# tencent-ailab/V-Express

Measured on NVIDIA H100. Metric: frames_per_sec_512x512_25step, higher is better.
Workload: dtype bf16

## Files before the change

### v-express_b200/csrc/vx_flash_attn.cu

```cuda
#include "vx_host.h"
#include "vx_ptx.cuh"

namespace vx {

constexpr int kFaRows = 64;
constexpr int kFaThreads = 128;

struct FaArgs {
  int Nq, Nk, hd, kv_div, stages;
  float scale_log2;
  __nv_bfloat16* out;
  long long ldo;
};

template <int HDP>
__global__ void __launch_bounds__(kFaThreads)
flash_attn_wgmma_kernel(const __grid_constant__ CUtensorMap mapQ, const __grid_constant__ CUtensorMap mapK,
                        const __grid_constant__ CUtensorMap mapV, const FaArgs p) {
  constexpr int kTile = kFaRows * HDP * 2;
  extern __shared__ uint8_t smem_raw[];
  uint8_t* smem = reinterpret_cast<uint8_t*>((reinterpret_cast<uintptr_t>(smem_raw) + 127) & ~uintptr_t(127));
  uint8_t* sQ = smem;
  uint8_t* sK = sQ + kTile;
  uint8_t* sV = sK + p.stages * kTile;
  uint64_t* q_full = reinterpret_cast<uint64_t*>(sV + p.stages * kTile);
  uint64_t* kv_full = q_full + 1;

  const int warp = threadIdx.x >> 5, lane = threadIdx.x & 31;
  const int q_tile = blockIdx.x, head = blockIdx.y, bq = blockIdx.z;
  const int T = (p.Nk + kFaRows - 1) / kFaRows;
  if (HDP > p.hd) {
    uint4* z = reinterpret_cast<uint4*>(sQ);
    for (int i = threadIdx.x; i < (1 + 2 * p.stages) * kTile / 16; i += blockDim.x) z[i] = make_uint4(0, 0, 0, 0);
  }
  if (threadIdx.x == 0) {
    mbar_init(q_full, 1);
    for (int s = 0; s < p.stages; ++s) mbar_init(&kv_full[s], 1);
    fence_barrier_init();
  }
  fence_proxy_async_smem();
  __syncthreads();
  pdl_wait();

  const int col_chunk = head * p.hd / 8;
  const int kv_row0 = (bq / p.kv_div) * p.Nk;
  auto load_kv = [&](int j) {
    const int st = j % p.stages;
    mbar_expect_tx(&kv_full[st], 2 * kFaRows * p.hd * 2);
    tma_load_3d(sK + st * kTile, &mapK, &kv_full[st], 0, kv_row0 + j * kFaRows, col_chunk);
    tma_load_3d(sV + st * kTile, &mapV, &kv_full[st], 0, kv_row0 + j * kFaRows, col_chunk);
  };
  if (threadIdx.x == 0) {
    tma_prefetch_desc(&mapQ);
    tma_prefetch_desc(&mapK);
    tma_prefetch_desc(&mapV);
    mbar_expect_tx(q_full, kFaRows * p.hd * 2);
    tma_load_3d(sQ, &mapQ, q_full, 0, bq * p.Nq + q_tile * kFaRows, col_chunk);
    for (int j = 0; j < p.stages && j < T; ++j) load_kv(j);
  }

  const uint64_t dq = make_smem_desc(smem_u32(sQ), kFaRows * 16, 128, SWZ_NONE);
  const float c = p.scale_log2;
  float o[HDP / 2];
#pragma unroll
  for (int i = 0; i < HDP / 2; ++i) o[i] = 0.f;
  float m_run[2] = {-INFINITY, -INFINITY}, l[2] = {0.f, 0.f};
  const int cq = (lane & 3) * 2;
  mbar_wait(q_full, 0);
  for (int j = 0; j < T; ++j) {
    const int st = j % p.stages;
    mbar_wait(&kv_full[st], (uint32_t)((j / p.stages) & 1));
    float s[32];
    const uint64_t dk = make_smem_desc(smem_u32(sK + st * kTile), kFaRows * 16, 128, SWZ_NONE);
    wgmma_fence();
#pragma unroll
    for (int k = 0; k < HDP / 16; ++k) Wgmma<64>::ss<0, 0>(s, dq + (uint64_t)(k * 128), dk + (uint64_t)(k * 128), k);
    wgmma_commit();
    wgmma_wait<0>();
    wgmma_fence_regs(s);
    if ((j + 1) * kFaRows > p.Nk) {
#pragma unroll
      for (int i = 0; i < 32; ++i)
        if (j * kFaRows + (i >> 2) * 8 + cq + (i & 1) >= p.Nk) s[i] = -INFINITY;
    }
    float alpha[2], mc[2];
#pragma unroll
    for (int h = 0; h < 2; ++h) {
      float mx = -INFINITY;
#pragma unroll
      for (int g = 0; g < 8; ++g) mx = fmaxf(mx, fmaxf(s[4 * g + 2 * h], s[4 * g + 2 * h + 1]));
      mx = fmaxf(mx, __shfl_xor_sync(0xffffffffu, mx, 1));
      mx = fmaxf(mx, __shfl_xor_sync(0xffffffffu, mx, 2));
      const float m_new = fmaxf(m_run[h], mx);
      alpha[h] = m_run[h] == -INFINITY ? 0.f : exp2f((m_run[h] - m_new) * c);
      m_run[h] = m_new;
      mc[h] = m_new * c;
      l[h] *= alpha[h];
    }
#pragma unroll
    for (int i = 0; i < HDP / 2; ++i) o[i] *= alpha[(i >> 1) & 1];
    uint32_t pa[4][4];
#pragma unroll
    for (int i = 0; i < 32; i += 2) {
      const int h = (i >> 1) & 1;
      const float e0 = exp2f(fmaf(s[i], c, -mc[h])), e1 = exp2f(fmaf(s[i + 1], c, -mc[h]));
      l[h] += e0 + e1;
      pa[i >> 3][(i >> 1) & 3] = pack_bf16(e0, e1);
    }
    const uint64_t dv = make_smem_desc(smem_u32(sV + st * kTile), 128, kFaRows * 16, SWZ_NONE);
    wgmma_fence();
#pragma unroll
    for (int k = 0; k < kFaRows / 16; ++k) Wgmma<HDP>::template rs<1>(o, pa[k], dv + (uint64_t)(k * 16), 1);
    wgmma_commit();
    wgmma_wait<0>();
    wgmma_fence_regs(o);
    __syncthreads();
    if (threadIdx.x == 0 && j + p.stages < T) load_kv(j + p.stages);
  }
#pragma unroll
  for (int h = 0; h < 2; ++h) {
    float lt = l[h];
    lt += __shfl_xor_sync(0xffffffffu, lt, 1);
    lt += __shfl_xor_sync(0xffffffffu, lt, 2);
    const float inv = 1.f / lt;
    const int qrow = q_tile * kFaRows + warp * 16 + (lane >> 2) + 8 * h;
    if (qrow < p.Nq) {
      __nv_bfloat16* op = p.out + ((long long)bq * p.Nq + qrow) * p.ldo + head * p.hd;
#pragma unroll
      for (int g = 0; g < HDP / 8; ++g)
        if (g * 8 + cq < p.hd)
          *reinterpret_cast<uint32_t*>(op + g * 8 + cq) = pack_bf16(o[4 * g + 2 * h] * inv, o[4 * g + 2 * h + 1] * inv);
    }
  }
}

constexpr int kFaPipeMaxHd = 56;
constexpr int kFaPipeStages = 4;

template <int HD, int NCONS>
__global__ void __launch_bounds__(128 * (NCONS + 1), 2)
flash_attn_pipe_kernel(const __grid_constant__ CUtensorMap mapQ, const __grid_constant__ CUtensorMap mapK,
                       const __grid_constant__ CUtensorMap mapV, const FaArgs p) {
  constexpr int HDP = (HD + 15) / 16 * 16;
  constexpr int kTile = kFaRows * HDP * 2;
  extern __shared__ uint8_t smem_raw[];
  uint8_t* smem = reinterpret_cast<uint8_t*>((reinterpret_cast<uintptr_t>(smem_raw) + 127) & ~uintptr_t(127));
  uint8_t* sQ = smem;
  uint8_t* sK = sQ + NCONS * kTile;
  uint8_t* sV = sK + p.stages * kTile;
  uint64_t* q_full = reinterpret_cast<uint64_t*>(sV + p.stages * kTile);
  uint64_t* kv_full = q_full + 1;
  uint64_t* kv_empty = kv_full + p.stages;

  const int warp = threadIdx.x >> 5, lane = threadIdx.x & 31;
  const int q_tile = blockIdx.x, head = blockIdx.y, bq = blockIdx.z;
  const int T = (p.Nk + kFaRows - 1) / kFaRows;
  if (HDP > HD) {
    uint4* z = reinterpret_cast<uint4*>(sQ);
    for (int i = threadIdx.x; i < (NCONS + 2 * p.stages) * kTile / 16; i += blockDim.x) z[i] = make_uint4(0, 0, 0, 0);
  }
  if (threadIdx.x == 0) {
    mbar_init(q_full, 1);
    for (int s = 0; s < p.stages; ++s) {
      mbar_init(&kv_full[s], 1);
      mbar_init(&kv_empty[s], 4 * NCONS);
    }
    fence_barrier_init();
  }
  fence_proxy_async_smem();
  __syncthreads();
  pdl_wait();

  const int col_chunk = head * HD / 8;
  if (warp < 4) {
    if (NCONS == 2) setmaxnreg_dec<24>();
    if (warp == 0 && lane == 0) {
      tma_prefetch_desc(&mapQ);
      tma_prefetch_desc(&mapK);
      tma_prefetch_desc(&mapV);
      mbar_expect_tx(q_full, NCONS * kFaRows * HD * 2);
      for (int w = 0; w < NCONS; ++w)
        tma_load_3d(sQ + w * kTile, &mapQ, q_full, 0, bq * p.Nq + (q_tile * NCONS + w) * kFaRows, col_chunk);
      const int kv_row0 = (bq / p.kv_div) * p.Nk;
      int st = 0;
      uint32_t phase = 0;
      for (int j = 0; j < T; ++j) {
        if (j >= p.stages) mbar_wait(&kv_empty[st], phase ^ 1);
        mbar_expect_tx(&kv_full[st], 2 * kFaRows * HD * 2);
        tma_load_3d(sK + st * kTile, &mapK, &kv_full[st], 0, kv_row0 + j * kFaRows, col_chunk);
        tma_load_3d(sV + st * kTile, &mapV, &kv_full[st], 0, kv_row0 + j * kFaRows, col_chunk);
        if (++st == p.stages) {
          st = 0;
          phase ^= 1;
        }
      }
    }
    return;
  }
  if (NCONS == 2) setmaxnreg_inc<104>();
  const int wg = (warp >> 2) - 1;
  const uint64_t dq = make_smem_desc(smem_u32(sQ + wg * kTile), kFaRows * 16, 128, SWZ_NONE);
  const float c = p.scale_log2;
  const int cq = (lane & 3) * 2;
  float o[HD / 2], s[32];
  uint32_t pa[4][4];
#pragma unroll
  for (int i = 0; i < HD / 2; ++i) o[i] = 0.f;
  float m_run[2] = {-INFINITY, -INFINITY}, l[2] = {0.f, 0.f}, alpha[2];

  auto issue_s = [&](int st) {
    const uint64_t dk = make_smem_desc(smem_u32(sK + st * kTile), kFaRows * 16, 128, SWZ_NONE);
#pragma unroll
    for (int k = 0; k < HDP / 16; ++k) Wgmma<64>::ss<0, 0>(s, dq + (uint64_t)(k * 128), dk + (uint64_t)(k * 128), k);
    wgmma_commit();
  };
  auto softmax = [&](int j) {
    if ((j + 1) * kFaRows > p.Nk) {
#pragma unroll
      for (int i = 0; i < 32; ++i)
        if (j * kFaRows + (i >> 2) * 8 + cq + (i & 1) >= p.Nk) s[i] = -INFINITY;
    }
    float mc[2];
#pragma unroll
    for (int h = 0; h < 2; ++h) {
      float mx = -INFINITY;
#pragma unroll
      for (int g = 0; g < 8; ++g) mx = fmaxf(mx, fmaxf(s[4 * g + 2 * h], s[4 * g + 2 * h + 1]));
      mx = fmaxf(mx, __shfl_xor_sync(0xffffffffu, mx, 1));
      mx = fmaxf(mx, __shfl_xor_sync(0xffffffffu, mx, 2));
      const float m_new = fmaxf(m_run[h], mx);
      alpha[h] = ex2_ftz(__fmul_rn(__fsub_rn(m_run[h], m_new), c));
      m_run[h] = m_new;
      mc[h] = __fmul_rn(m_new, c);
    }
#pragma unroll
    for (int i = 0; i < 32; i += 2) {
      const int h = (i >> 1) & 1;
      s[i] = ex2_ftz(__fmaf_rn(s[i], c, -mc[h]));
      s[i + 1] = ex2_ftz(__fmaf_rn(s[i + 1], c, -mc[h]));
      const float e = __fadd_rn(s[i], s[i + 1]);
      l[h] = i < 4 ? __fmaf_rn(l[h], alpha[h], e) : __fadd_rn(l[h], e);
    }
  };
  auto pack = [&]() {
#pragma unroll
    for (int i = 0; i < 32; i += 2) pa[i >> 3][(i >> 1) & 3] = pack_bf16(s[i], s[i + 1]);
  };

  mbar_wait(q_full, 0);
  mbar_wait(&kv_full[0], 0);
  wgmma_fence();
  issue_s(0);
  wgmma_wait<0>();
  wgmma_fence_regs(s);
  softmax(0);
  pack();
  auto issue_pv = [&](int st) {
    const uint64_t dv = make_smem_desc(smem_u32(sV + st * kTile), 128, kFaRows * 16, SWZ_NONE);
#pragma unroll
    for (int k = 0; k < kFaRows / 16; ++k) Wgmma<HD>::template rs<1>(o, pa[k], dv + (uint64_t)(k * 16), 1);
    wgmma_commit();
  };
  auto pv_done = [&](int st) {
    wgmma_fence_regs(o);
#pragma unroll
    for (int k = 0; k < 4; ++k) wgmma_fence_regs(pa[k]);
    if (lane == 0) mbar_arrive(&kv_empty[st]);
  };
  int st = 0;
  uint32_t phase = 0;
  for (int j = 0; j + 1 < T; ++j) {
    int st1 = st + 1;
    uint32_t phase1 = phase;
    if (st1 == p.stages) {
      st1 = 0;
      phase1 ^= 1;
    }
    mbar_wait(&kv_full[st1], phase1);
    wgmma_fence();
    issue_s(st1);
    issue_pv(st);
    wgmma_wait<1>();
    wgmma_fence_regs(s);
    softmax(j + 1);
    wgmma_wait<0>();
    pv_done(st);
#pragma unroll
    for (int i = 0; i < HD / 2; ++i) o[i] = __fmul_rn(o[i], alpha[(i >> 1) & 1]);
    pack();
    st = st1;
    phase = phase1;
  }
  wgmma_fence();
  issue_pv(st);
  wgmma_wait<0>();
  pv_done(st);
#pragma unroll
  for (int h = 0; h < 2; ++h) {
    float lt = l[h];
    lt += __shfl_xor_sync(0xffffffffu, lt, 1);
    lt += __shfl_xor_sync(0xffffffffu, lt, 2);
    const float inv = 1.f / lt;
    const int qrow = (q_tile * NCONS + wg) * kFaRows + (warp & 3) * 16 + (lane >> 2) + 8 * h;
    if (qrow < p.Nq) {
      __nv_bfloat16* op = p.out + ((long long)bq * p.Nq + qrow) * p.ldo + head * HD;
#pragma unroll
      for (int g = 0; g < HD / 8; ++g)
        *reinterpret_cast<uint32_t*>(op + g * 8 + cq) = pack_bf16(o[4 * g + 2 * h] * inv, o[4 * g + 2 * h + 1] * inv);
    }
  }
}

template <auto Kernel>
static cudaError_t launch_fa(dim3 grid, int threads, size_t smem, cudaStream_t st, const CUtensorMap& mQ,
                             const CUtensorMap& mK, const CUtensorMap& mV, const FaArgs& a) {
  static bool configured = false;
  if (!configured) {
    const cudaError_t e = cudaFuncSetAttribute(Kernel, cudaFuncAttributeMaxDynamicSharedMemorySize, 227 * 1024);
    if (e != cudaSuccess) return e;
    configured = true;
  }
  return launch_k(Kernel, grid, dim3(threads), smem, st, mQ, mK, mV, a);
}

struct GaArgs {
  const __nv_bfloat16* q; long long ldq;
  const __nv_bfloat16* k; long long ldk;
  const __nv_bfloat16* v; long long ldv;
  __nv_bfloat16* out; long long ldo;
  int Bq, Nq, Nk, heads, hd, kv_div;
  float scale;
};

__global__ void __launch_bounds__(128) generic_attn_kernel(const GaArgs p) {
  pdl_enter();
  extern __shared__ float sc_all[];
  const int warp = threadIdx.x >> 5, lane = threadIdx.x & 31;
  float* sc = sc_all + warp * p.Nk;
  const long long item = (long long)blockIdx.x * 4 + warp;
  const long long total = (long long)p.Bq * p.heads * p.Nq;
  if (item >= total) return;
  const int qi = (int)(item % p.Nq);
  const int head = (int)((item / p.Nq) % p.heads);
  const int b = (int)(item / ((long long)p.Nq * p.heads));
  const __nv_bfloat16* qp = p.q + ((long long)b * p.Nq + qi) * p.ldq + head * p.hd;
  const long long kv0 = (long long)(b / p.kv_div) * p.Nk;
  float mx = -INFINITY;
  for (int j = lane; j < p.Nk; j += 32) {
    const __nv_bfloat16* kp = p.k + (kv0 + j) * p.ldk + head * p.hd;
    float acc = 0.f;
    for (int c = 0; c < p.hd; c += 2) {
      const float2 a = __bfloat1622float2(*reinterpret_cast<const __nv_bfloat162*>(qp + c));
      const float2 bb = __bfloat1622float2(*reinterpret_cast<const __nv_bfloat162*>(kp + c));
      acc += a.x * bb.x + a.y * bb.y;
    }
    acc *= p.scale;
    sc[j] = acc;
    mx = fmaxf(mx, acc);
  }
  for (int o = 16; o; o >>= 1) mx = fmaxf(mx, __shfl_xor_sync(0xffffffffu, mx, o));
  float sum = 0.f;
  for (int j = lane; j < p.Nk; j += 32) {
    const float e = __expf(sc[j] - mx);
    sc[j] = e;
    sum += e;
  }
  for (int o = 16; o; o >>= 1) sum += __shfl_xor_sync(0xffffffffu, sum, o);
  __syncwarp();
  const float inv = 1.f / sum;
  for (int c = lane * 2; c < p.hd; c += 64) {
    float o0 = 0.f, o1 = 0.f;
    for (int j = 0; j < p.Nk; ++j) {
      const float2 vv = __bfloat1622float2(*reinterpret_cast<const __nv_bfloat162*>(p.v + (kv0 + j) * p.ldv + head * p.hd + c));
      o0 += sc[j] * vv.x;
      o1 += sc[j] * vv.y;
    }
    *reinterpret_cast<__nv_bfloat162*>(p.out + ((long long)b * p.Nq + qi) * p.ldo + head * p.hd + c) =
        __floats2bfloat162_rn(o0 * inv, o1 * inv);
  }
}

}

using namespace vx;

static bool& fa_v1() {
  static bool v = getenv("VX_FA_V1") != nullptr;
  return v;
}
extern "C" void vx_flash_reload_env() { fa_v1() = getenv("VX_FA_V1") != nullptr; }

extern "C" int vx_flash_attention(const void* q, long long ldq, const void* k, long long ldk, const void* v,
                                  long long ldv, void* out, long long ldo, int Bq, int Nq, int Bkv, int Nk, int heads,
                                  int hd, int kv_div, void* stream) {
  VX_REQUIRE(hd % 8 == 0 && hd <= 256, "vx_flash_attention: hd=%d unsupported", hd);
  VX_REQUIRE(ldq % 8 == 0 && ldk % 8 == 0 && ldv % 8 == 0 && ldo % 8 == 0, "vx_flash_attention: ld must be %%8");
  VX_REQUIRE(kv_div >= 1 && (Bq + kv_div - 1) / kv_div <= Bkv, "vx_flash_attention: kv_div=%d Bq=%d Bkv=%d", kv_div, Bq, Bkv);
  if (Nk < 16 || Nk % 16 != 0) {
    VX_REQUIRE(Nk * 4 * 4 <= 48 * 1024, "vx_flash_attention: Nk=%d not a multiple of 16 and too long for the fallback", Nk);
    GaArgs g{(const __nv_bfloat16*)q, ldq, (const __nv_bfloat16*)k, ldk, (const __nv_bfloat16*)v, ldv,
             (__nv_bfloat16*)out, ldo, Bq, Nq, Nk, heads, hd, kv_div, 1.0f / sqrtf((float)hd)};
    const long long items = (long long)Bq * heads * Nq;
    launch_k(generic_attn_kernel, dim3((unsigned)((items + 3) / 4)), dim3(128), (size_t)Nk * 4 * 4, (cudaStream_t)stream, g);
    VX_CHECK_CUDA(cudaGetLastError());
    return 0;
  }
  const int hdp = (hd + 15) / 16 * 16;
  const bool pipe = hd <= kFaPipeMaxHd && !fa_v1();
  const int ncons = pipe && Nq > kFaRows ? 2 : 1;
  const int stages = pipe ? kFaPipeStages : hdp > 96 ? 2 : 3;
  const size_t smem = (size_t)(ncons + 2 * stages) * kFaRows * hdp * 2 + 128 + 128;
  CUtensorMap mQ, mK, mV;
  const void* ptrs[3] = {q, k, v};
  const long long lds[3] = {ldq, ldk, ldv};
  const long long rows[3] = {(long long)Bq * Nq, (long long)Bkv * Nk, (long long)Bkv * Nk};
  CUtensorMap* maps[3] = {&mQ, &mK, &mV};
  for (int i = 0; i < 3; ++i) {
    uint64_t dims[3] = {8, (uint64_t)rows[i], (uint64_t)lds[i] / 8};
    uint64_t str[2] = {(uint64_t)lds[i] * 2, 16};
    uint32_t box[3] = {8, (uint32_t)kFaRows, (uint32_t)hd / 8};
    if (make_tmap_bf16(maps[i], ptrs[i], 3, dims, str, box, CU_TENSOR_MAP_SWIZZLE_NONE)) return 1;
  }
  FaArgs a{};
  a.Nq = Nq; a.Nk = Nk; a.hd = hd; a.kv_div = kv_div; a.stages = stages;
  a.scale_log2 = 1.4426950408889634f / sqrtf((float)hd);
  a.out = (__nv_bfloat16*)out; a.ldo = ldo;
  const dim3 grid((Nq + ncons * kFaRows - 1) / (ncons * kFaRows), heads, Bq);
  if (pipe) {
    const cudaStream_t cs = (cudaStream_t)stream;
    cudaError_t e;
    switch (hd) {
#define VX_FA_CASE(H)                                                                                       \
    case H:                                                                                                 \
      if (ncons == 2) e = launch_fa<flash_attn_pipe_kernel<H, 2>>(grid, 384, smem, cs, mQ, mK, mV, a);         \
      else e = launch_fa<flash_attn_pipe_kernel<H, 1>>(grid, 256, smem, cs, mQ, mK, mV, a);                    \
      break;
      VX_FA_CASE(8) VX_FA_CASE(16) VX_FA_CASE(24) VX_FA_CASE(32) VX_FA_CASE(40) VX_FA_CASE(48) VX_FA_CASE(56)
#undef VX_FA_CASE
      default: return fail("vx_flash_attention: hd=%d unsupported", hd);
    }
    VX_CHECK_CUDA(e);
    VX_CHECK_CUDA(cudaGetLastError());
    return 0;
  }
  switch (hdp) {
#define VX_FA_CASE(H) \
    case H: VX_CHECK_CUDA(launch_fa<flash_attn_wgmma_kernel<H>>(grid, kFaThreads, smem, (cudaStream_t)stream, mQ, mK, mV, a)); break;
    VX_FA_CASE(16) VX_FA_CASE(32) VX_FA_CASE(48) VX_FA_CASE(64) VX_FA_CASE(80) VX_FA_CASE(96) VX_FA_CASE(112) VX_FA_CASE(128)
    VX_FA_CASE(144) VX_FA_CASE(160) VX_FA_CASE(176) VX_FA_CASE(192) VX_FA_CASE(208) VX_FA_CASE(224) VX_FA_CASE(240)
    VX_FA_CASE(256)
#undef VX_FA_CASE
    default: return fail("vx_flash_attention: hd=%d unsupported", hd);
  }
  VX_CHECK_CUDA(cudaGetLastError());
  return 0;
}
```

Before: 5.443.

## Extend warp-specialized flash attention to hd 80/160 and add three-consumer ping-pong path

Extends the producer/consumer TMA-pipelined attention kernel to head dims 80 and 160, which are typical of UNet attention layers in this model. For small head dims with long queries it uses three consumer warpgroups, double-buffering the score registers so the next QK^T GEMM is already issued while softmax runs on the current tile. Register budgets, CTAs per SM and ring depth are now computed from the head dim and consumer count instead of being fixed. The cost is higher register pressure and shared-memory use, and occupancy drops to one CTA per SM for the multi-consumer variants.

```diff
diff --git a/v-express_b200/csrc/vx_flash_attn.cu b/v-express_b200/csrc/vx_flash_attn.cu
--- a/v-express_b200/csrc/vx_flash_attn.cu
+++ b/v-express_b200/csrc/vx_flash_attn.cu
@@ -134,11 +134,24 @@
   }
 }
 
-constexpr int kFaPipeMaxHd = 56;
-constexpr int kFaPipeStages = 4;
+constexpr bool fa_pipe_hd(int hd) { return hd % 8 == 0 && (hd <= 56 || hd == 80 || hd == 160); }
+constexpr int fa_pipe_ncons(int hd, int Nq) { return Nq <= kFaRows ? 1 : hd <= 56 ? 3 : 2; }
+constexpr int fa_pipe_ctas(int ncons) { return ncons == 1 ? 2 : 1; }
+constexpr int fa_pipe_consumer_regs(int ncons) {
+  const int pool = 65536 / (fa_pipe_ctas(ncons) * 128 * (ncons + 1)) / 8 * 8 * (ncons + 1);
+  const int r = (pool - 24) / ncons / 8 * 8;
+  return r < 232 ? r : 232;
+}
+constexpr int fa_pipe_stages(int hd, int ncons) {
+  const int tile = kFaRows * ((hd + 15) / 16 * 16) * 2;
+  const int per_cta = 228 * 1024 / fa_pipe_ctas(ncons) - 1024 - 256;
+  const int s = (per_cta - ncons * tile) / (2 * tile);
+  return s < 4 ? s : 4;
+}
+static_assert(fa_pipe_stages(160, 1) >= 2 && fa_pipe_stages(160, 2) == 4 && fa_pipe_stages(56, 3) == 4, "ring depth");
 
 template <int HD, int NCONS>
-__global__ void __launch_bounds__(128 * (NCONS + 1), 2)
+__global__ void __launch_bounds__(128 * (NCONS + 1), fa_pipe_ctas(NCONS))
 flash_attn_pipe_kernel(const __grid_constant__ CUtensorMap mapQ, const __grid_constant__ CUtensorMap mapK,
                        const __grid_constant__ CUtensorMap mapV, const FaArgs p) {
   constexpr int HDP = (HD + 15) / 16 * 16;
@@ -173,7 +186,7 @@
 
   const int col_chunk = head * HD / 8;
   if (warp < 4) {
-    if (NCONS == 2) setmaxnreg_dec<24>();
+    setmaxnreg_dec<24>();
     if (warp == 0 && lane == 0) {
       tma_prefetch_desc(&mapQ);
       tma_prefetch_desc(&mapK);
@@ -197,7 +210,7 @@
     }
     return;
   }
-  if (NCONS == 2) setmaxnreg_inc<104>();
+  setmaxnreg_inc<fa_pipe_consumer_regs(NCONS)>();
   const int wg = (warp >> 2) - 1;
   const uint64_t dq = make_smem_desc(smem_u32(sQ + wg * kTile), kFaRows * 16, 128, SWZ_NONE);
   const float c = p.scale_log2;
@@ -208,13 +221,13 @@
   for (int i = 0; i < HD / 2; ++i) o[i] = 0.f;
   float m_run[2] = {-INFINITY, -INFINITY}, l[2] = {0.f, 0.f}, alpha[2];
 
-  auto issue_s = [&](int st) {
+  auto issue_s = [&](float (&s)[32], int st) {
     const uint64_t dk = make_smem_desc(smem_u32(sK + st * kTile), kFaRows * 16, 128, SWZ_NONE);
 #pragma unroll
     for (int k = 0; k < HDP / 16; ++k) Wgmma<64>::ss<0, 0>(s, dq + (uint64_t)(k * 128), dk + (uint64_t)(k * 128), k);
     wgmma_commit();
   };
-  auto softmax = [&](int j) {
+  auto softmax = [&](float (&s)[32], int j) {
     if ((j + 1) * kFaRows > p.Nk) {
 #pragma unroll
       for (int i = 0; i < 32; ++i)
@@ -242,33 +255,101 @@
       l[h] = i < 4 ? __fmaf_rn(l[h], alpha[h], e) : __fadd_rn(l[h], e);
     }
   };
-  auto pack = [&]() {
+  auto pack = [&](const float (&s)[32]) {
 #pragma unroll
     for (int i = 0; i < 32; i += 2) pa[i >> 3][(i >> 1) & 3] = pack_bf16(s[i], s[i + 1]);
   };
 
+  auto issue_pv = [&](int st) {
+    const uint64_t dv = make_smem_desc(smem_u32(sV + st * kTile), 128, kFaRows * 16, SWZ_NONE);
+#pragma unroll
+    for (int k = 0; k < kFaRows / 16; ++k) Wgmma<HD>::template rs<1>(o, pa[k], dv + (uint64_t)(k * 16), 1);
+    wgmma_commit();
+  };
+  auto pv_done = [&](int st) {
+    wgmma_fence_regs(o);
+#pragma unroll
+    for (int k = 0; k < 4; ++k) wgmma_fence_regs(pa[k]);
+    if (lane == 0) mbar_arrive(&kv_empty[st]);
+  };
+  auto rescale = [&]() {
+#pragma unroll
+    for (int i = 0; i < HD / 2; ++i) o[i] = __fmul_rn(o[i], alpha[(i >> 1) & 1]);
+  };
   mbar_wait(q_full, 0);
+  int st = 0;
+  uint32_t phase = 0;
+  if constexpr (NCONS == 3) {
+    float s2[32];
+    int ist = 0;
+    uint32_t iph = 0;
+    auto next_s = [&](float (&sx)[32]) {
+      mbar_wait(&kv_full[ist], iph);
+      wgmma_fence();
+      issue_s(sx, ist);
+      if (++ist == p.stages) {
+        ist = 0;
+        iph ^= 1;
+      }
+    };
+    auto step = [&](float (&cur)[32], float (&nxt)[32], int j) {
+      wgmma_fence();
+      issue_pv(st);
+      next_s(nxt);
+      wgmma_wait<2>();
+      wgmma_fence_regs(cur);
+      softmax(cur, j + 1);
+      wgmma_wait<1>();
+      pv_done(st);
+      rescale();
+      pack(cur);
+      if (++st == p.stages) st = 0;
+    };
+    auto last = [&](float (&cur)[32], int j) {
+      wgmma_fence();
+      issue_pv(st);
+      wgmma_wait<1>();
+      wgmma_fence_regs(cur);
+      softmax(cur, j + 1);
+      wgmma_wait<0>();
+      pv_done(st);
+      rescale();
+      pack(cur);
+      if (++st == p.stages) st = 0;
+    };
+    next_s(s);
+    if (T == 1) {
+      wgmma_wait<0>();
+      wgmma_fence_regs(s);
+      softmax(s, 0);
+      pack(s);
+    } else {
+      next_s(s2);
+      wgmma_wait<1>();
+      wgmma_fence_regs(s);
+      softmax(s, 0);
+      pack(s);
+      for (int j = 0;; j += 2) {
+        if (j + 2 >= T) {
+          last(s2, j);
+          break;
+        }
+        step(s2, s, j);
+        if (j + 3 >= T) {
+          last(s, j + 1);
+          break;
+        }
+        step(s, s2, j + 1);
+      }
+    }
+  } else {
   mbar_wait(&kv_full[0], 0);
   wgmma_fence();
-  issue_s(0);
+  issue_s(s, 0);
   wgmma_wait<0>();
   wgmma_fence_regs(s);
-  softmax(0);
-  pack();
-  auto issue_pv = [&](int st) {
-    const uint64_t dv = make_smem_desc(smem_u32(sV + st * kTile), 128, kFaRows * 16, SWZ_NONE);
-#pragma unroll
-    for (int k = 0; k < kFaRows / 16; ++k) Wgmma<HD>::template rs<1>(o, pa[k], dv + (uint64_t)(k * 16), 1);
-    wgmma_commit();
-  };
-  auto pv_done = [&](int st) {
-    wgmma_fence_regs(o);
-#pragma unroll
-    for (int k = 0; k < 4; ++k) wgmma_fence_regs(pa[k]);
-    if (lane == 0) mbar_arrive(&kv_empty[st]);
-  };
-  int st = 0;
-  uint32_t phase = 0;
+  softmax(s, 0);
+  pack(s);
   for (int j = 0; j + 1 < T; ++j) {
     int st1 = st + 1;
     uint32_t phase1 = phase;
@@ -278,18 +359,18 @@
     }
     mbar_wait(&kv_full[st1], phase1);
     wgmma_fence();
-    issue_s(st1);
+    issue_s(s, st1);
     issue_pv(st);
     wgmma_wait<1>();
     wgmma_fence_regs(s);
-    softmax(j + 1);
+    softmax(s, j + 1);
     wgmma_wait<0>();
     pv_done(st);
-#pragma unroll
-    for (int i = 0; i < HD / 2; ++i) o[i] = __fmul_rn(o[i], alpha[(i >> 1) & 1]);
-    pack();
+    rescale();
+    pack(s);
     st = st1;
     phase = phase1;
+  }
   }
   wgmma_fence();
   issue_pv(st);
@@ -406,9 +487,9 @@
     return 0;
   }
   const int hdp = (hd + 15) / 16 * 16;
-  const bool pipe = hd <= kFaPipeMaxHd && !fa_v1();
-  const int ncons = pipe && Nq > kFaRows ? 2 : 1;
-  const int stages = pipe ? kFaPipeStages : hdp > 96 ? 2 : 3;
+  const bool pipe = fa_pipe_hd(hd) && !fa_v1();
+  const int ncons = pipe ? fa_pipe_ncons(hd, Nq) : 1;
+  const int stages = pipe ? fa_pipe_stages(hd, ncons) : hdp > 96 ? 2 : 3;
   const size_t smem = (size_t)(ncons + 2 * stages) * kFaRows * hdp * 2 + 128 + 128;
   CUtensorMap mQ, mK, mV;
   const void* ptrs[3] = {q, k, v};
@@ -432,10 +513,13 @@
     switch (hd) {
 #define VX_FA_CASE(H)                                                                                       \
     case H:                                                                                                 \
-      if (ncons == 2) e = launch_fa<flash_attn_pipe_kernel<H, 2>>(grid, 384, smem, cs, mQ, mK, mV, a);         \
+      if (ncons == fa_pipe_ncons(H, kFaRows + 1))                                                           \
+        e = launch_fa<flash_attn_pipe_kernel<H, fa_pipe_ncons(H, kFaRows + 1)>>(grid, 128 * (ncons + 1), smem, cs, mQ, \
+                                                                             mK, mV, a);                 \
       else e = launch_fa<flash_attn_pipe_kernel<H, 1>>(grid, 256, smem, cs, mQ, mK, mV, a);                    \
       break;
       VX_FA_CASE(8) VX_FA_CASE(16) VX_FA_CASE(24) VX_FA_CASE(32) VX_FA_CASE(40) VX_FA_CASE(48) VX_FA_CASE(56)
+      VX_FA_CASE(80) VX_FA_CASE(160)
 #undef VX_FA_CASE
       default: return fail("vx_flash_attention: hd=%d unsupported", hd);
     }
```

Result: faster. 5.615, median of 6 (+3.2%).
